# facebookresearch/flashy

Measured on AMD Instinct MI355X. Metric: img/sec, higher is better.
Workload: dtype bf16; 1 GPU; model=resnet18, dataset=cifar10-shaped, global_batch=64, img_size=32, num_classes=10, parallelism=dp1, mode=native-kernels, graph=True, channels_last=False

## Files before the change

### flashy_amd/ops/csrc/conv_wgrad.hip

```cpp

#include "conv_common.h"

#define WG_P 72

__global__ void __launch_bounds__(CONV_THREADS, 4)
k_conv_wgrad(const uint16_t* __restrict__ x, const uint16_t* __restrict__ dout,
             float* __restrict__ dw, ConvDims d, int m_per_split) {
    const int rsc = d.R * d.S * d.C;
    const int64_t M = (int64_t)d.N * d.Ho * d.Wo;
    const int tid = threadIdx.x;
    const int lane = tid & 63;
    const int wid = tid >> 6;
    const int wave_k = wid >> 1;
    const int wave_j = wid & 1;
    const int k0 = blockIdx.x * 64;
    const int j0 = blockIdx.y * 64;
    const int64_t ms = (int64_t)blockIdx.z * m_per_split;
    const int64_t me = min(ms + (int64_t)m_per_split, M);

    __shared__ __attribute__((aligned(16))) uint16_t doutT[2][2 * 32 * WG_P];
    __shared__ __attribute__((aligned(16))) uint16_t xT[2][2 * 32 * WG_P];

    floatx4 acc[2][2] = {};

    const int m_r = tid >> 3;
    const int k8 = (tid & 7) * 8;
    const int t_r = (j0 + k8) / (d.S * d.C);
    const int t_scc = (j0 + k8) - t_r * d.S * d.C;
    const int t_s = t_scc / d.C;
    const int t_c = t_scc - t_s * d.C;
    const int t_hoff = t_r - d.pad;
    const int t_woff = t_s - d.pad;
    auto load_pair = [&](int64_t mc, short8* dv, short8* xv) {
#pragma unroll
        for (int sc = 0; sc < 2; ++sc) {
            const int64_t m = mc + sc * CONV_BK + m_r;
            short8 v = {};
            if (m < me)
                v = *reinterpret_cast<const short8*>(dout + m * d.K + k0 + k8);
            dv[sc] = v;
            short8 u = {};
            if (m < me) {
                const int wo = (int)(m % d.Wo);
                const int ho = (int)((m / d.Wo) % d.Ho);
                const int64_t n = m / ((int64_t)d.Ho * d.Wo);
                const int hi = ho * d.stride + t_hoff;
                const int wi = wo * d.stride + t_woff;
                if (hi >= 0 && hi < d.H && wi >= 0 && wi < d.W)
                    u = *reinterpret_cast<const short8*>(
                        x + (((n * d.H + hi) * d.W + wi) * (int64_t)d.C + t_c));
            }
            xv[sc] = u;
        }
    };
    auto stage_write = [&](uint16_t (&dT)[2 * 32 * WG_P],
                           uint16_t (&xTb)[2 * 32 * WG_P],
                           const short8* dv, const short8* xv) {
#pragma unroll
        for (int sc = 0; sc < 2; ++sc) {
            const int at = (sc * 32 + m_r) * WG_P + k8;
            *reinterpret_cast<short8*>(&dT[at]) = dv[sc];
            *reinterpret_cast<short8*>(&xTb[at]) = xv[sc];
        }
    };

    const int tr_lane = ((lane & 15) >> 2) * WG_P + 4 * (lane & 3) +
                        (lane >> 4) * 8 * WG_P;
    union U64x2 { struct { unsigned long long lo, hi; } q; short8 v; };

    const int64_t n_stages = (me - ms + 2 * CONV_BK - 1) / (2 * CONV_BK);
    short8 dv[2], xv[2];
    load_pair(ms, dv, xv);
    stage_write(doutT[0], xT[0], dv, xv);
    if (n_stages > 1) load_pair(ms + 2 * CONV_BK, dv, xv);
    __syncthreads();

    auto step = [&](int64_t i, const uint16_t (&dT)[2 * 32 * WG_P],
                    const uint16_t (&xTb)[2 * 32 * WG_P],
                    uint16_t (&ndT)[2 * 32 * WG_P],
                    uint16_t (&nxT)[2 * 32 * WG_P]) {
        if (i + 1 < n_stages) {
            stage_write(ndT, nxT, dv, xv);
            if (i + 2 < n_stages) load_pair(ms + (i + 2) * 2 * CONV_BK, dv, xv);
        }
        const unsigned a0 = (unsigned)(unsigned long long)(const void*)
            &dT[tr_lane + wave_k * 32];
        const unsigned a1 = a0 + 32;
        const unsigned b0 = (unsigned)(unsigned long long)(const void*)
            &xTb[tr_lane + wave_j * 32];
        const unsigned b1 = b0 + 32;
        U64x2 af[2][2], bf[2][2];
        asm volatile(
            "ds_read_b64_tr_b16 %0, %16\n\t"
            "ds_read_b64_tr_b16 %1, %16 offset:576\n\t"
            "ds_read_b64_tr_b16 %2, %17\n\t"
            "ds_read_b64_tr_b16 %3, %17 offset:576\n\t"
            "ds_read_b64_tr_b16 %4, %18\n\t"
            "ds_read_b64_tr_b16 %5, %18 offset:576\n\t"
            "ds_read_b64_tr_b16 %6, %19\n\t"
            "ds_read_b64_tr_b16 %7, %19 offset:576\n\t"
            "ds_read_b64_tr_b16 %8, %16 offset:4608\n\t"
            "ds_read_b64_tr_b16 %9, %16 offset:5184\n\t"
            "ds_read_b64_tr_b16 %10, %17 offset:4608\n\t"
            "ds_read_b64_tr_b16 %11, %17 offset:5184\n\t"
            "ds_read_b64_tr_b16 %12, %18 offset:4608\n\t"
            "ds_read_b64_tr_b16 %13, %18 offset:5184\n\t"
            "ds_read_b64_tr_b16 %14, %19 offset:4608\n\t"
            "ds_read_b64_tr_b16 %15, %19 offset:5184\n\t"
            "s_waitcnt lgkmcnt(8)"
            : "=&v"(af[0][0].q.lo), "=&v"(af[0][0].q.hi),
              "=&v"(af[0][1].q.lo), "=&v"(af[0][1].q.hi),
              "=&v"(bf[0][0].q.lo), "=&v"(bf[0][0].q.hi),
              "=&v"(bf[0][1].q.lo), "=&v"(bf[0][1].q.hi),
              "=&v"(af[1][0].q.lo), "=&v"(af[1][0].q.hi),
              "=&v"(af[1][1].q.lo), "=&v"(af[1][1].q.hi),
              "=&v"(bf[1][0].q.lo), "=&v"(bf[1][0].q.hi),
              "=&v"(bf[1][1].q.lo), "=&v"(bf[1][1].q.hi)
            : "v"(a0), "v"(a1), "v"(b0), "v"(b1));
#pragma unroll
        for (int kf = 0; kf < 2; ++kf)
#pragma unroll
            for (int jf = 0; jf < 2; ++jf)
                acc[kf][jf] = MFMA_BF16(af[0][kf].v, bf[0][jf].v, acc[kf][jf]);
        asm volatile("s_waitcnt lgkmcnt(0)"
                     : "+v"(af[1][0].q.lo), "+v"(af[1][0].q.hi),
                       "+v"(af[1][1].q.lo), "+v"(af[1][1].q.hi),
                       "+v"(bf[1][0].q.lo), "+v"(bf[1][0].q.hi),
                       "+v"(bf[1][1].q.lo), "+v"(bf[1][1].q.hi));
        __builtin_amdgcn_sched_barrier(0);
#pragma unroll
        for (int kf = 0; kf < 2; ++kf)
#pragma unroll
            for (int jf = 0; jf < 2; ++jf)
                acc[kf][jf] = MFMA_BF16(af[1][kf].v, bf[1][jf].v, acc[kf][jf]);
        __syncthreads();
    };
    for (int64_t i = 0; i < n_stages;) {
        step(i, doutT[0], xT[0], doutT[1], xT[1]);
        if (++i >= n_stages) break;
        step(i, doutT[1], xT[1], doutT[0], xT[0]);
        ++i;
    }

    const int out_k0 = k0 + wave_k * 32 + (lane >> 4) * 4;
    const int out_j0 = j0 + wave_j * 32 + (lane & 15);
#pragma unroll
    for (int kf = 0; kf < 2; ++kf)
#pragma unroll
        for (int jf = 0; jf < 2; ++jf)
#pragma unroll
            for (int rr = 0; rr < 4; ++rr) {
                const int k = out_k0 + kf * 16 + rr;
                const int j = out_j0 + jf * 16;
                atomicAdd(&dw[(int64_t)k * rsc + j], acc[kf][jf][rr]);
            }
}


#define WG_P8 144

__global__ void __launch_bounds__(512, 2)
k_conv_wgrad8(const uint16_t* __restrict__ x, const uint16_t* __restrict__ dout,
              float* __restrict__ dw, ConvDims d, int m_per_split) {
    const int rsc = d.R * d.S * d.C;
    const int64_t M = (int64_t)d.N * d.Ho * d.Wo;
    const int tid = threadIdx.x;
    const int lane = tid & 63;
    const int wid = tid >> 6;
    const int wave_k = wid >> 2;
    const int wave_j = wid & 3;
    const int k0 = blockIdx.x * 128;
    const int j0 = blockIdx.y * 128;
    const int64_t ms = (int64_t)blockIdx.z * m_per_split;
    const int64_t me = min(ms + (int64_t)m_per_split, M);

    __shared__ __attribute__((aligned(16))) uint16_t doutT[2][2 * 32 * WG_P8];
    __shared__ __attribute__((aligned(16))) uint16_t xT[2][2 * 32 * WG_P8];

    floatx4 acc[4][2] = {};

    const int m_r = tid >> 3;
    const int k8 = (tid & 7) * 8;
    int t_hoff[2], t_woff[2], t_c[2];
#pragma unroll
    for (int h = 0; h < 2; ++h) {
        const int jj = j0 + h * 64 + k8;
        const int r = jj / (d.S * d.C);
        const int scc = jj - r * d.S * d.C;
        const int s = scc / d.C;
        t_c[h] = scc - s * d.C;
        t_hoff[h] = r - d.pad;
        t_woff[h] = s - d.pad;
    }
    auto load_pair = [&](int64_t mc, short8* dv, short8* xv) {
        const int64_t m = mc + m_r;
        short8 z = {};
        dv[0] = dv[1] = xv[0] = xv[1] = z;
        if (m < me) {
            dv[0] = *reinterpret_cast<const short8*>(dout + m * d.K + k0 + k8);
            dv[1] = *reinterpret_cast<const short8*>(
                dout + m * d.K + k0 + 64 + k8);
            const int wo = (int)(m % d.Wo);
            const int ho = (int)((m / d.Wo) % d.Ho);
            const int64_t n = m / ((int64_t)d.Ho * d.Wo);
#pragma unroll
            for (int h = 0; h < 2; ++h) {
                const int hi = ho * d.stride + t_hoff[h];
                const int wi = wo * d.stride + t_woff[h];
                if (hi >= 0 && hi < d.H && wi >= 0 && wi < d.W)
                    xv[h] = *reinterpret_cast<const short8*>(
                        x + (((n * d.H + hi) * d.W + wi) * (int64_t)d.C +
                             t_c[h]));
            }
        }
    };
    auto stage_write = [&](uint16_t (&dT)[2 * 32 * WG_P8],
                           uint16_t (&xTb)[2 * 32 * WG_P8],
                           const short8* dv, const short8* xv) {
        const int at = m_r * WG_P8 + k8;
#pragma unroll
        for (int h = 0; h < 2; ++h) {
            *reinterpret_cast<short8*>(&dT[at + h * 64]) = dv[h];
            *reinterpret_cast<short8*>(&xTb[at + h * 64]) = xv[h];
        }
    };

    const int tr_lane = ((lane & 15) >> 2) * WG_P8 + 4 * (lane & 3) +
                        (lane >> 4) * 8 * WG_P8;
    union U64x2 { struct { unsigned long long lo, hi; } q; short8 v; };

    const int64_t n_stages = (me - ms + 2 * CONV_BK - 1) / (2 * CONV_BK);
    short8 dv[2], xv[2];
    load_pair(ms, dv, xv);
    stage_write(doutT[0], xT[0], dv, xv);
    if (n_stages > 1) load_pair(ms + 2 * CONV_BK, dv, xv);
    __syncthreads();

    auto step = [&](int64_t i, const uint16_t (&dT)[2 * 32 * WG_P8],
                    const uint16_t (&xTb)[2 * 32 * WG_P8],
                    uint16_t (&ndT)[2 * 32 * WG_P8],
                    uint16_t (&nxT)[2 * 32 * WG_P8]) {
        if (i + 1 < n_stages) {
            stage_write(ndT, nxT, dv, xv);
            if (i + 2 < n_stages) load_pair(ms + (i + 2) * 2 * CONV_BK, dv, xv);
        }
        const unsigned a0 = (unsigned)(unsigned long long)(const void*)
            &dT[tr_lane + wave_k * 64];
        const unsigned b0 = (unsigned)(unsigned long long)(const void*)
            &xTb[tr_lane + wave_j * 32];
        U64x2 af[2][4], bf[2][2];
#pragma unroll
        for (int sc = 0; sc < 2; ++sc) {
            asm volatile(
                "ds_read_b64_tr_b16 %0, %12\n\t"
                "ds_read_b64_tr_b16 %1, %12 offset:1152\n\t"
                "ds_read_b64_tr_b16 %2, %12 offset:32\n\t"
                "ds_read_b64_tr_b16 %3, %12 offset:1184\n\t"
                "ds_read_b64_tr_b16 %4, %12 offset:64\n\t"
                "ds_read_b64_tr_b16 %5, %12 offset:1216\n\t"
                "ds_read_b64_tr_b16 %6, %12 offset:96\n\t"
                "ds_read_b64_tr_b16 %7, %12 offset:1248\n\t"
                "ds_read_b64_tr_b16 %8, %13\n\t"
                "ds_read_b64_tr_b16 %9, %13 offset:1152\n\t"
                "ds_read_b64_tr_b16 %10, %13 offset:32\n\t"
                "ds_read_b64_tr_b16 %11, %13 offset:1184\n\t"
                : "=&v"(af[sc][0].q.lo), "=&v"(af[sc][0].q.hi),
                  "=&v"(af[sc][1].q.lo), "=&v"(af[sc][1].q.hi),
                  "=&v"(af[sc][2].q.lo), "=&v"(af[sc][2].q.hi),
                  "=&v"(af[sc][3].q.lo), "=&v"(af[sc][3].q.hi),
                  "=&v"(bf[sc][0].q.lo), "=&v"(bf[sc][0].q.hi),
                  "=&v"(bf[sc][1].q.lo), "=&v"(bf[sc][1].q.hi)
                : "v"(a0 + sc * 9216), "v"(b0 + sc * 9216));
        }
#pragma unroll
        for (int sc = 0; sc < 2; ++sc) {
            if (sc == 0)
                asm volatile("s_waitcnt lgkmcnt(12)"
                             : "+v"(af[0][0].q.lo), "+v"(af[0][0].q.hi),
                               "+v"(af[0][1].q.lo), "+v"(af[0][1].q.hi),
                               "+v"(af[0][2].q.lo), "+v"(af[0][2].q.hi),
                               "+v"(af[0][3].q.lo), "+v"(af[0][3].q.hi),
                               "+v"(bf[0][0].q.lo), "+v"(bf[0][0].q.hi),
                               "+v"(bf[0][1].q.lo), "+v"(bf[0][1].q.hi));
            else
                asm volatile("s_waitcnt lgkmcnt(0)"
                             : "+v"(af[1][0].q.lo), "+v"(af[1][0].q.hi),
                               "+v"(af[1][1].q.lo), "+v"(af[1][1].q.hi),
                               "+v"(af[1][2].q.lo), "+v"(af[1][2].q.hi),
                               "+v"(af[1][3].q.lo), "+v"(af[1][3].q.hi),
                               "+v"(bf[1][0].q.lo), "+v"(bf[1][0].q.hi),
                               "+v"(bf[1][1].q.lo), "+v"(bf[1][1].q.hi));
            __builtin_amdgcn_sched_barrier(0);
#pragma unroll
            for (int kf = 0; kf < 4; ++kf)
#pragma unroll
                for (int jf = 0; jf < 2; ++jf)
                    acc[kf][jf] =
                        MFMA_BF16(af[sc][kf].v, bf[sc][jf].v, acc[kf][jf]);
        }
        __syncthreads();
    };
    for (int64_t i = 0; i < n_stages;) {
        step(i, doutT[0], xT[0], doutT[1], xT[1]);
        if (++i >= n_stages) break;
        step(i, doutT[1], xT[1], doutT[0], xT[0]);
        ++i;
    }

    const int out_k0 = k0 + wave_k * 64 + (lane >> 4) * 4;
    const int out_j0 = j0 + wave_j * 32 + (lane & 15);
#pragma unroll
    for (int kf = 0; kf < 4; ++kf)
#pragma unroll
        for (int jf = 0; jf < 2; ++jf)
#pragma unroll
            for (int rr = 0; rr < 4; ++rr) {
                const int k = out_k0 + kf * 16 + rr;
                const int j = out_j0 + jf * 16;
                atomicAdd(&dw[(int64_t)k * rsc + j], acc[kf][jf][rr]);
            }
}

extern "C" void launch_conv_wgrad(const void* x, const void* dout, void* dw,
                                  ConvDims d, int n_splits, hipStream_t stream) {
    const int rsc = d.R * d.S * d.C;
    const int64_t M = (int64_t)d.N * d.Ho * d.Wo;
    const int tiles8 = (d.K / 128) * (rsc / 128);
    const bool wg8 = d.R * d.S > 1 && d.K % 128 == 0 && rsc % 128 == 0 &&
                     (M >= 32768 || (M >= 8192 && tiles8 >= 18) ||
                      tiles8 >= 100);
    if (wg8) {
        const int tiles = (d.K / 128) * (rsc / 128);
        int ns = n_splits;
        if (ns > 1) {
            ns = 512 / tiles;
            if (ns < 1) ns = 1;
            if (ns > 128) ns = 128;
            const int64_t mcap = M / 64;
            if (ns > mcap) ns = (int)(mcap ? mcap : 1);
        }
        int mps = (int)((M + ns - 1) / ns);
        mps = (mps + 2 * CONV_BK - 1) / (2 * CONV_BK) * (2 * CONV_BK);
        const int zn = (int)((M + mps - 1) / mps);
        dim3 grid((unsigned)(d.K / 128), (unsigned)(rsc / 128), (unsigned)zn);
        k_conv_wgrad8<<<grid, 512, 0, stream>>>(
            (const uint16_t*)x, (const uint16_t*)dout, (float*)dw, d, mps);
        return;
    }
    int m_per_split = (int)((M + n_splits - 1) / n_splits);
    m_per_split = (m_per_split + 2 * CONV_BK - 1) / (2 * CONV_BK) * (2 * CONV_BK);
    const int zn = (int)((M + m_per_split - 1) / m_per_split);
    dim3 grid((unsigned)(d.K / 64), (unsigned)(rsc / 64), (unsigned)zn);
    k_conv_wgrad<<<grid, CONV_THREADS, 0, stream>>>(
        (const uint16_t*)x, (const uint16_t*)dout, (float*)dw, d, m_per_split);
}
```

Baseline: 30300 img/s.

## Group multiple M-split ranges per block and reduce wgrad partials in LDS

The 64x64 wgrad kernel is templated on MG, which packs MG split-K groups into one block. Each group accumulates its own M range, the partial tiles are summed through shared memory, and the result is issued as a single atomicAdd per element, cutting global atomic traffic. When only one split exists, both kernels use a plain read-modify-write instead of atomics. A heuristic picks MG from tile count, occupancy and range length. The cost is larger dynamic LDS per block and an added sync and reduction pass.

```diff
diff --git a/flashy_amd/ops/csrc/conv_wgrad.hip b/flashy_amd/ops/csrc/conv_wgrad.hip
--- a/flashy_amd/ops/csrc/conv_wgrad.hip
+++ b/flashy_amd/ops/csrc/conv_wgrad.hip
@@ -2,24 +2,35 @@
 #include "conv_common.h"
 
 #define WG_P 72
-
-__global__ void __launch_bounds__(CONV_THREADS, 4)
+#define WG_STAGE (2 * 32 * WG_P)
+#define WG_GROUP_ELEMS (4 * WG_STAGE)
+#define WG_GROUP_BYTES (WG_GROUP_ELEMS * 2)
+#define WG_TP 68
+
+template <int MG>
+__global__ void __launch_bounds__(CONV_THREADS * MG, 4)
 k_conv_wgrad(const uint16_t* __restrict__ x, const uint16_t* __restrict__ dout,
-             float* __restrict__ dw, ConvDims d, int m_per_split) {
+             float* __restrict__ dw, ConvDims d, int m_per_split, int single) {
     const int rsc = d.R * d.S * d.C;
     const int64_t M = (int64_t)d.N * d.Ho * d.Wo;
-    const int tid = threadIdx.x;
+    const int grp = threadIdx.x / CONV_THREADS;
+    const int tid = threadIdx.x % CONV_THREADS;
     const int lane = tid & 63;
     const int wid = tid >> 6;
     const int wave_k = wid >> 1;
     const int wave_j = wid & 1;
     const int k0 = blockIdx.x * 64;
     const int j0 = blockIdx.y * 64;
-    const int64_t ms = (int64_t)blockIdx.z * m_per_split;
+    const int64_t ms0 = (int64_t)blockIdx.z * MG * m_per_split;
+    const int64_t ms = min(ms0 + (int64_t)grp * m_per_split, M);
     const int64_t me = min(ms + (int64_t)m_per_split, M);
 
-    __shared__ __attribute__((aligned(16))) uint16_t doutT[2][2 * 32 * WG_P];
-    __shared__ __attribute__((aligned(16))) uint16_t xT[2][2 * 32 * WG_P];
+    extern __shared__ __attribute__((aligned(16))) uint16_t wg_lds[];
+    uint16_t* const gbase = wg_lds + grp * WG_GROUP_ELEMS;
+    uint16_t* const doutT0 = gbase;
+    uint16_t* const doutT1 = gbase + WG_STAGE;
+    uint16_t* const xT0 = gbase + 2 * WG_STAGE;
+    uint16_t* const xT1 = gbase + 3 * WG_STAGE;
 
     floatx4 acc[2][2] = {};
 
@@ -53,8 +64,7 @@
             xv[sc] = u;
         }
     };
-    auto stage_write = [&](uint16_t (&dT)[2 * 32 * WG_P],
-                           uint16_t (&xTb)[2 * 32 * WG_P],
+    auto stage_write = [&](uint16_t* dT, uint16_t* xTb,
                            const short8* dv, const short8* xv) {
 #pragma unroll
         for (int sc = 0; sc < 2; ++sc) {
@@ -68,17 +78,17 @@
                         (lane >> 4) * 8 * WG_P;
     union U64x2 { struct { unsigned long long lo, hi; } q; short8 v; };
 
-    const int64_t n_stages = (me - ms + 2 * CONV_BK - 1) / (2 * CONV_BK);
+    const int64_t n_stages =
+        (min(ms0 + (int64_t)m_per_split, M) - ms0 + 2 * CONV_BK - 1) /
+        (2 * CONV_BK);
     short8 dv[2], xv[2];
     load_pair(ms, dv, xv);
-    stage_write(doutT[0], xT[0], dv, xv);
+    stage_write(doutT0, xT0, dv, xv);
     if (n_stages > 1) load_pair(ms + 2 * CONV_BK, dv, xv);
     __syncthreads();
 
-    auto step = [&](int64_t i, const uint16_t (&dT)[2 * 32 * WG_P],
-                    const uint16_t (&xTb)[2 * 32 * WG_P],
-                    uint16_t (&ndT)[2 * 32 * WG_P],
-                    uint16_t (&nxT)[2 * 32 * WG_P]) {
+    auto step = [&](int64_t i, const uint16_t* dT, const uint16_t* xTb,
+                    uint16_t* ndT, uint16_t* nxT) {
         if (i + 1 < n_stages) {
             stage_write(ndT, nxT, dv, xv);
             if (i + 2 < n_stages) load_pair(ms + (i + 2) * 2 * CONV_BK, dv, xv);
@@ -136,24 +146,50 @@
         __syncthreads();
     };
     for (int64_t i = 0; i < n_stages;) {
-        step(i, doutT[0], xT[0], doutT[1], xT[1]);
+        step(i, doutT0, xT0, doutT1, xT1);
         if (++i >= n_stages) break;
-        step(i, doutT[1], xT[1], doutT[0], xT[0]);
+        step(i, doutT1, xT1, doutT0, xT0);
         ++i;
     }
 
-    const int out_k0 = k0 + wave_k * 32 + (lane >> 4) * 4;
-    const int out_j0 = j0 + wave_j * 32 + (lane & 15);
+    const int t_k = wave_k * 32 + (lane >> 4) * 4;
+    const int t_j = wave_j * 32 + (lane & 15);
+    if constexpr (MG == 1) {
+        if (!single) {
+#pragma unroll
+            for (int kf = 0; kf < 2; ++kf)
+#pragma unroll
+                for (int jf = 0; jf < 2; ++jf)
+#pragma unroll
+                    for (int rr = 0; rr < 4; ++rr)
+                        atomicAdd(&dw[(int64_t)(k0 + t_k + kf * 16 + rr) * rsc +
+                                      j0 + t_j + jf * 16],
+                                  acc[kf][jf][rr]);
+            return;
+        }
+    }
+    float* const tile = reinterpret_cast<float*>(gbase);
 #pragma unroll
     for (int kf = 0; kf < 2; ++kf)
 #pragma unroll
         for (int jf = 0; jf < 2; ++jf)
 #pragma unroll
-            for (int rr = 0; rr < 4; ++rr) {
-                const int k = out_k0 + kf * 16 + rr;
-                const int j = out_j0 + jf * 16;
-                atomicAdd(&dw[(int64_t)k * rsc + j], acc[kf][jf][rr]);
-            }
+            for (int rr = 0; rr < 4; ++rr)
+                tile[(t_k + kf * 16 + rr) * WG_TP + t_j + jf * 16] =
+                    acc[kf][jf][rr];
+    __syncthreads();
+    const float* const tiles = reinterpret_cast<const float*>(wg_lds);
+    for (int r = threadIdx.x >> 6; r < 64; r += 4 * MG) {
+        float v = tiles[r * WG_TP + lane];
+#pragma unroll
+        for (int g = 1; g < MG; ++g)
+            v += tiles[g * (WG_GROUP_BYTES / 4) + r * WG_TP + lane];
+        float* const p = &dw[(int64_t)(k0 + r) * rsc + j0 + lane];
+        if (single)
+            *p += v;
+        else
+            atomicAdd(p, v);
+    }
 }
 
 
@@ -161,7 +197,7 @@
 
 __global__ void __launch_bounds__(512, 2)
 k_conv_wgrad8(const uint16_t* __restrict__ x, const uint16_t* __restrict__ dout,
-              float* __restrict__ dw, ConvDims d, int m_per_split) {
+              float* __restrict__ dw, ConvDims d, int m_per_split, int single) {
     const int rsc = d.R * d.S * d.C;
     const int64_t M = (int64_t)d.N * d.Ho * d.Wo;
     const int tid = threadIdx.x;
@@ -317,8 +353,60 @@
             for (int rr = 0; rr < 4; ++rr) {
                 const int k = out_k0 + kf * 16 + rr;
                 const int j = out_j0 + jf * 16;
-                atomicAdd(&dw[(int64_t)k * rsc + j], acc[kf][jf][rr]);
+                float* const p = &dw[(int64_t)k * rsc + j];
+                if (single)
+                    *p += acc[kf][jf][rr];
+                else
+                    atomicAdd(p, acc[kf][jf][rr]);
             }
+}
+
+#include <cstdlib>
+static int wgrad_mg_forced() {
+    const char* e = getenv("FLASHY_WGRAD_MG");
+    if (e && (e[0] == '1' || e[0] == '2' || e[0] == '4') && !e[1])
+        return e[0] - '0';
+    return 0;
+}
+
+static int wgrad_pick_mg(int tiles, int ranges, int m_per_split) {
+    if (m_per_split > 32 * CONV_BK) return 1;
+    const int64_t blocks1 = (int64_t)tiles * ranges;
+    const int64_t rounds1 = (blocks1 + 1023) / 1024;
+    const int64_t fill1 = blocks1 < 256 ? blocks1 : 256;
+    const bool short_range = m_per_split <= 4 * CONV_BK;
+    for (int mg = 4; mg > 1; mg >>= 1) {
+        if (mg > ranges) continue;
+        const int zn = (ranges + mg - 1) / mg;
+        const int64_t blocks = (int64_t)tiles * zn;
+        const int64_t slots = 1024 / mg;
+        const bool fits = blocks <= slots * rounds1 + (mg == 2 ? slots / 8 : 0);
+        const bool padded = (mg * zn - ranges) * 5 > ranges;
+        const bool filled = short_range ? blocks * 2 >= fill1
+                                        : blocks * 10 >= fill1 * 9;
+        if (fits && !padded && filled) return mg;
+    }
+    return 1;
+}
+
+template <int MG>
+static void launch_wgrad_mg(const void* x, const void* dout, void* dw,
+                            const ConvDims& d, int m_per_split, int ranges,
+                            hipStream_t stream) {
+    constexpr int lds = MG * WG_GROUP_BYTES;
+    static const bool attr_set = [] {
+        (void)hipFuncSetAttribute((const void*)&k_conv_wgrad<MG>,
+                                  hipFuncAttributeMaxDynamicSharedMemorySize,
+                                  lds);
+        return true;
+    }();
+    (void)attr_set;
+    const int zn = (ranges + MG - 1) / MG;
+    dim3 grid((unsigned)(d.K / 64), (unsigned)(d.R * d.S * d.C / 64),
+              (unsigned)zn);
+    k_conv_wgrad<MG><<<grid, CONV_THREADS * MG, lds, stream>>>(
+        (const uint16_t*)x, (const uint16_t*)dout, (float*)dw, d, m_per_split,
+        zn == 1);
 }
 
 extern "C" void launch_conv_wgrad(const void* x, const void* dout, void* dw,
@@ -344,13 +432,20 @@
         const int zn = (int)((M + mps - 1) / mps);
         dim3 grid((unsigned)(d.K / 128), (unsigned)(rsc / 128), (unsigned)zn);
         k_conv_wgrad8<<<grid, 512, 0, stream>>>(
-            (const uint16_t*)x, (const uint16_t*)dout, (float*)dw, d, mps);
+            (const uint16_t*)x, (const uint16_t*)dout, (float*)dw, d, mps,
+            zn == 1);
         return;
     }
     int m_per_split = (int)((M + n_splits - 1) / n_splits);
     m_per_split = (m_per_split + 2 * CONV_BK - 1) / (2 * CONV_BK) * (2 * CONV_BK);
-    const int zn = (int)((M + m_per_split - 1) / m_per_split);
-    dim3 grid((unsigned)(d.K / 64), (unsigned)(rsc / 64), (unsigned)zn);
-    k_conv_wgrad<<<grid, CONV_THREADS, 0, stream>>>(
-        (const uint16_t*)x, (const uint16_t*)dout, (float*)dw, d, m_per_split);
-}
+    const int ranges = (int)((M + m_per_split - 1) / m_per_split);
+    const int tiles = (d.K / 64) * (rsc / 64);
+    int mg = wgrad_mg_forced();
+    if (!mg) mg = wgrad_pick_mg(tiles, ranges, m_per_split);
+    if (mg == 4)
+        launch_wgrad_mg<4>(x, dout, dw, d, m_per_split, ranges, stream);
+    else if (mg == 2)
+        launch_wgrad_mg<2>(x, dout, dw, d, m_per_split, ranges, stream);
+    else
+        launch_wgrad_mg<1>(x, dout, dw, d, m_per_split, ranges, stream);
+}
```

After: 30860 img/s (median of 6 runs). 1.02x the previous value.
